# alehdaghi/vq-vae-2-pytorch

Measured on AMD Instinct MI355X. Metric: images/sec VQ-VAE-2 256px train step, higher is better.
Workload: dtype f32; 1 GPU; configs[1]: 256x256 FFHQ-shaped synthetic, default two-level VQ-VAE-2, batch 32/GPU; global_batch=32, image=256, n_embed=512, parallelism=dp1

## Files before the change

### vq-vae-2-pytorch_amd/csrc/vq2_resblock.hip

```cpp
#include "vq2_common.h"
#include "vq2_rbwino.h"

namespace vq2 {

typedef unsigned int u32x4 __attribute__((ext_vector_type(4)));

namespace rb {
constexpr unsigned RSRC_FLAGS = 0x00020000;
constexpr int OOB = 0x7F000000;
constexpr int TH = 8, TW = 16;
constexpr int PW = TW + 2, PH = TH + 2;
constexpr int NPATCH = PW * PH;
constexpr int CS = 16;
constexpr int LDK = CS + 4;
constexpr int CM = 32;
constexpr int CC = 128;
constexpr int A_F4 = NPATCH * CS / 4;
constexpr int B_F4 = 9 * CM * CS / 4;
constexpr int A_FLOATS = ((A_F4 + 255) / 256) * 64 * LDK;
constexpr int B_FLOATS = ((B_F4 + 255) / 256) * 64 * LDK;
constexpr int LDR = CM + 4;
constexpr size_t LDS_BYTES = (size_t)2 * (A_FLOATS + B_FLOATS) * sizeof(float);
static_assert(2 * LDS_BYTES <= 160 * 1024, "two workgroups per CU");
static_assert(128 * LDR <= 2 * (A_FLOATS + B_FLOATS), "stage-2 aliases fit in the stage-1 buffers");
}

struct ResFwdParams {
    const float *x;
    const float *w1;
    const float *b1;
    const float *w2;
    const float *b2;
    float *r;
    float *y;
    int N, H, W, ldx, ldr, ldy;
    int tiles_x, tiles_y;
    int relu_out;
};

__device__ __forceinline__ float4 u4_as_f4(u32x4 v) {
    return make_float4(__uint_as_float(v.x), __uint_as_float(v.y), __uint_as_float(v.z), __uint_as_float(v.w));
}

__global__ __launch_bounds__(256, 2) void resblock_fwd_kernel(const ResFwdParams P) {
    using namespace rb;
    constexpr int NT = 256;
    constexpr int A_LD = (A_F4 + NT - 1) / NT;
    constexpr int B_LD = (B_F4 + NT - 1) / NT;
    constexpr int NS = CC / CS;
    constexpr int NJ = CC / 32;
    extern __shared__ __attribute__((aligned(16))) float smem[];
    float *As = smem;
    float *Bs = smem + 2 * A_FLOATS;
    float *Rs = smem;

    const int tid = threadIdx.x, lane = tid & 63, wave = tid >> 6;
    const int wq = wave;
    const int l31 = lane & 31, fk = 4 * (lane >> 5);
    const int tiles = P.tiles_x * P.tiles_y;
    const int vid = xcd_remap(blockIdx.x, gridDim.x);
    const int n = vid / tiles;
    const int t = vid - n * tiles;
    const int tyi = t / P.tiles_x;
    const int y0 = tyi * TH, x0 = (t - tyi * P.tiles_x) * TW;

    const int npix = P.N * P.H * P.W;
    const __amdgpu_buffer_rsrc_t rx = __builtin_amdgcn_make_buffer_rsrc(const_cast<float *>(P.x), 0, npix * P.ldx * 4, RSRC_FLAGS);
    const __amdgpu_buffer_rsrc_t rw1 = __builtin_amdgcn_make_buffer_rsrc(const_cast<float *>(P.w1), 0, CM * 9 * CC * 4, RSRC_FLAGS);
    const __amdgpu_buffer_rsrc_t rw2 = __builtin_amdgcn_make_buffer_rsrc(const_cast<float *>(P.w2), 0, CC * CM * 4, RSRC_FLAGS);

    int a_off[A_LD], b_off[B_LD];
#pragma unroll
    for (int j = 0; j < A_LD; ++j) {
        const int f = tid + NT * j;
        a_off[j] = OOB;
        if (f < A_F4) {
            const int pp = f >> 2;
            const int pr = pp / PW, pc = pp - pr * PW;
            const int gy = y0 - 1 + pr, gx = x0 - 1 + pc;
            if ((unsigned)gy < (unsigned)P.H && (unsigned)gx < (unsigned)P.W)
                a_off[j] = ((n * P.H + gy) * P.W + gx) * P.ldx * 4 + (f & 3) * 16;
        }
    }
#pragma unroll
    for (int j = 0; j < B_LD; ++j) {
        const int f = tid + NT * j;
        b_off[j] = OOB;
        if (f < B_F4) {
            const int row = f >> 2;
            b_off[j] = ((row & 31) * 9 * CC + (row >> 5) * CC) * 4 + (f & 3) * 16;
        }
    }
    const int st_off = (tid >> 2) * LDK + (tid & 3) * 4;
    struct Slice { u32x4 a[A_LD], b[B_LD]; };
    auto issue_loads = [&](int s, Slice &r) {
        const int soff = s * CS * 4;
#pragma unroll
        for (int j = 0; j < A_LD; ++j) r.a[j] = __builtin_amdgcn_raw_buffer_load_b128(rx, a_off[j], soff, 0);
#pragma unroll
        for (int j = 0; j < B_LD; ++j) r.b[j] = __builtin_amdgcn_raw_buffer_load_b128(rw1, b_off[j], soff, 0);
    };
    auto store_slice = [&](int buf, const Slice &r) {
        float *a = As + buf * A_FLOATS + st_off;
        float *b = Bs + buf * B_FLOATS + st_off;
#pragma unroll
        for (int j = 0; j < A_LD; ++j)
            *reinterpret_cast<float4 *>(a + j * (NT / 4) * LDK) = relu4(u4_as_f4(r.a[j]));
#pragma unroll
        for (int j = 0; j < B_LD; ++j)
            *reinterpret_cast<float4 *>(b + j * (NT / 4) * LDK) = u4_as_f4(r.b[j]);
    };

    f32x16 acc1;
#pragma unroll
    for (int r = 0; r < 16; ++r) acc1[r] = 0.f;

    const int a_frag = ((2 * wq + (l31 >> 4)) * PW + (l31 < 16 ? l31 : ((l31 + 14) & 15))) * LDK + fk;
    const int b_frag = l31 * LDK + fk;
    auto stage_one_store = [&](int buf, const Slice &r, int j) {
        if (j < A_LD) *reinterpret_cast<float4 *>(As + buf * A_FLOATS + st_off + j * (NT / 4) * LDK) = relu4(u4_as_f4(r.a[j]));
        else *reinterpret_cast<float4 *>(Bs + buf * B_FLOATS + st_off + (j - A_LD) * (NT / 4) * LDK) = u4_as_f4(r.b[j - A_LD]);
    };
    auto stage_one_load = [&](int s, Slice &r, int j) {
        if (j < A_LD) r.a[j] = __builtin_amdgcn_raw_buffer_load_b128(rx, a_off[j], s * CS * 4, 0);
        else r.b[j - A_LD] = __builtin_amdgcn_raw_buffer_load_b128(rw1, b_off[j - A_LD], s * CS * 4, 0);
    };
    int pix_lane;
    {
        const int gy = y0 + 2 * wq + (l31 >> 4), gx = x0 + (l31 < 16 ? l31 : ((l31 + 14) & 15));
        pix_lane = (gy < P.H && gx < P.W) ? (n * P.H + gy) * P.W + gx : -1;
    }
    const int rowq = 4 * (lane >> 5);
    int xoff[16], yoff[16];
#pragma unroll
    for (int r = 0; r < 16; ++r) {
        const int pix = __shfl(pix_lane, rowq + (r & 3) + 8 * (r >> 2), 64);
        xoff[r] = pix >= 0 ? pix * (P.ldx * 4) + l31 * 4 : OOB;
        yoff[r] = pix >= 0 ? pix * (P.ldy * 4) + l31 * 4 : OOB;
    }
    f32x16 acc2[NJ];
    float4 w2f[NJ][CM / 8];
    float b1v = 0.f, b2v[NJ];
    const __amdgpu_buffer_rsrc_t rb1 = __builtin_amdgcn_make_buffer_rsrc(const_cast<float *>(P.b1), 0, CM * 4, RSRC_FLAGS);
    const __amdgpu_buffer_rsrc_t rb2 = __builtin_amdgcn_make_buffer_rsrc(const_cast<float *>(P.b2), 0, CC * 4, RSRC_FLAGS);

    auto stage2_load = [&](int i) {
        constexpr int NW2 = NJ * (CM / 8);
        if (i < NW2) {
            const int j = i / (CM / 8), k8 = i % (CM / 8);
            w2f[j][k8] = u4_as_f4(__builtin_amdgcn_raw_buffer_load_b128(rw2, ((j * 32 + l31) * CM + fk + 8 * k8) * 4, 0, 0));
        } else if (i < NW2 + NJ * 16) {
            const int j = (i - NW2) / 16, r = (i - NW2) % 16;
            acc2[j][r] = __uint_as_float(__builtin_amdgcn_raw_buffer_load_b32(rx, xoff[r] + j * 128, 0, 0));
        } else if (i == NW2 + NJ * 16) {
            b1v = __uint_as_float(__builtin_amdgcn_raw_buffer_load_b32(rb1, l31 * 4, 0, 0));
        } else if (i <= NW2 + NJ * 16 + NJ) {
            const int j = i - (NW2 + NJ * 16 + 1);
            b2v[j] = __uint_as_float(__builtin_amdgcn_raw_buffer_load_b32(rb2, (j * 32 + l31) * 4, 0, 0));
        }
    };
    auto compute_staged = [&](int buf, int s, Slice &r, bool do_store, bool do_load, bool do_stage2) {
        const float *a0 = As + buf * A_FLOATS + a_frag;
        const float *b0 = Bs + buf * B_FLOATS + b_frag;
        constexpr int NP = 9 * (CS / 8);
        constexpr int NST = A_LD + B_LD;
        static_assert(2 * NST <= NP, "stores then loads fit in the MFMA groups of one slice");
        float4 fa[2], fb[2];
        fa[0] = *reinterpret_cast<const float4 *>(a0);
        fb[0] = *reinterpret_cast<const float4 *>(b0);
#pragma unroll
        for (int p = 0; p < NP; ++p) {
            const int cur = p & 1, nxt = cur ^ 1;
            if (p + 1 < NP) {
                const int tap = (p + 1) / (CS / 8), k8 = (p + 1) % (CS / 8);
                fa[nxt] = *reinterpret_cast<const float4 *>(a0 + ((tap / 3) * PW + (tap % 3)) * LDK + 8 * k8);
                fb[nxt] = *reinterpret_cast<const float4 *>(b0 + tap * 32 * LDK + 8 * k8);
            }
            acc1 = __builtin_amdgcn_mfma_f32_32x32x2f32(fa[cur].x, fb[cur].x, acc1, 0, 0, 0);
            acc1 = __builtin_amdgcn_mfma_f32_32x32x2f32(fa[cur].y, fb[cur].y, acc1, 0, 0, 0);
            acc1 = __builtin_amdgcn_mfma_f32_32x32x2f32(fa[cur].z, fb[cur].z, acc1, 0, 0, 0);
            acc1 = __builtin_amdgcn_mfma_f32_32x32x2f32(fa[cur].w, fb[cur].w, acc1, 0, 0, 0);
            if (p < NST) { if (do_store) stage_one_store(buf ^ 1, r, p); }
            __builtin_amdgcn_sched_group_barrier(0x100, 2, 0);
            __builtin_amdgcn_sched_group_barrier(0x008, 4, 0);
            if (p < NST) __builtin_amdgcn_sched_group_barrier(0x200, 1, 0);
            if (p >= NST && p < 2 * NST && do_load) {
                __builtin_amdgcn_sched_barrier(0);
                stage_one_load(s + 2, r, p - NST);
                __builtin_amdgcn_sched_barrier(0);
            }
            if (do_stage2) {
                constexpr int PER = (NJ * (CM / 8) + NJ * 16 + 1 + NJ + NP - 1) / NP;
                __builtin_amdgcn_sched_barrier(0);
#pragma unroll
                for (int q = 0; q < PER; ++q) stage2_load(p * PER + q);
                __builtin_amdgcn_sched_barrier(0);
            }
        }
    };

    Slice R0, R1;
    issue_loads(0, R0);
    issue_loads(1, R1);
    store_slice(0, R0);
    __syncthreads();
    store_slice(1, R1);
    __builtin_amdgcn_sched_barrier(0);
    compute_staged(0, 0, R0, false, true, false);
    __builtin_amdgcn_sched_barrier(0);
    __syncthreads();
    for (int s = 1; s < NS; ++s) {
        const int buf = s & 1;
        __builtin_amdgcn_sched_barrier(0);
        compute_staged(buf, s, R0, s + 1 < NS, s + 2 < NS, s + 1 == NS);
        __builtin_amdgcn_sched_barrier(0);
        __syncthreads();
    }
    const __amdgpu_buffer_rsrc_t rr = __builtin_amdgcn_make_buffer_rsrc(P.r, 0, npix * P.ldr * 4, RSRC_FLAGS);
    const __amdgpu_buffer_rsrc_t ry = __builtin_amdgcn_make_buffer_rsrc(P.y, 0, npix * P.ldy * 4, RSRC_FLAGS);
    float rv[16];
    int roff[16];
    {
        const int ldr4 = P.ldr * 4;
#pragma unroll
        for (int r = 0; r < 16; ++r) {
            const int row = rowq + (r & 3) + 8 * (r >> 2);
            const int pix = __shfl(pix_lane, row, 64);
            rv[r] = relu1(acc1[r] + b1v);
            Rs[(32 * wq + row) * LDR + l31] = rv[r];
            roff[r] = pix >= 0 ? pix * ldr4 + l31 * 4 : OOB;
        }
    }
    const int relu_floor_bits = P.relu_out ? 0 : (int)0x80000000;
    {
        const float *a = Rs + (32 * wq + l31) * LDR + fk;
        float4 fa[CM / 8];
#pragma unroll
        for (int k8 = 0; k8 < CM / 8; ++k8) fa[k8] = *reinterpret_cast<const float4 *>(a + 8 * k8);
#pragma unroll
        for (int j = 0; j < NJ; ++j) {
#pragma unroll
            for (int r = 0; r < 16; ++r) acc2[j][r] += b2v[j];
#pragma unroll
            for (int k8 = 0; k8 < CM / 8; ++k8) {
                const float4 fb = w2f[j][k8];
                acc2[j] = __builtin_amdgcn_mfma_f32_32x32x2f32(fa[k8].x, fb.x, acc2[j], 0, 0, 0);
                acc2[j] = __builtin_amdgcn_mfma_f32_32x32x2f32(fa[k8].y, fb.y, acc2[j], 0, 0, 0);
                acc2[j] = __builtin_amdgcn_mfma_f32_32x32x2f32(fa[k8].z, fb.z, acc2[j], 0, 0, 0);
                acc2[j] = __builtin_amdgcn_mfma_f32_32x32x2f32(fa[k8].w, fb.w, acc2[j], 0, 0, 0);
                __builtin_amdgcn_sched_barrier(0);
#pragma unroll
                for (int q = 0; q < 4; ++q) {
                    const int r = 4 * k8 + q;
                    if (j == 0) {
                        __builtin_amdgcn_raw_buffer_store_b32(__float_as_uint(rv[r]), rr, roff[r], 0, 0);
                    } else {
                        const float v = relu_floor(acc2[j - 1][r], relu_floor_bits);
                        __builtin_amdgcn_raw_buffer_store_b32(__float_as_uint(v), ry, yoff[r] + (j - 1) * 128, 0, 0);
                    }
                }
                __builtin_amdgcn_sched_barrier(0);
            }
        }
    }
#pragma unroll
    for (int r = 0; r < 16; ++r) {
        const float v = relu_floor(acc2[NJ - 1][r], relu_floor_bits);
        __builtin_amdgcn_raw_buffer_store_b32(__float_as_uint(v), ry, yoff[r] + (NJ - 1) * 128, 0, 0);
    }
}


namespace rbb {
using namespace rb;
constexpr int SA = 32;
constexpr int LDA = SA + 4;
constexpr int PROWS = 192;
constexpr int GA_FLOATS = PROWS * LDA;
constexpr int WA_FLOATS = CM * LDA;
constexpr int WB_FLOATS = CC * LDA;
constexpr size_t LDS_BYTES = (size_t)(2 * GA_FLOATS + 2 * WA_FLOATS) * sizeof(float);
constexpr int WR_FLOATS = 16 * 64 + 32;
constexpr size_t LDS_BYTES_W2 = LDS_BYTES + (size_t)4 * WR_FLOATS * sizeof(float);
static_assert(GA_FLOATS + 2 * WB_FLOATS <= 2 * GA_FLOATS + 2 * WA_FLOATS, "phase-B buffers alias the phase-A ones");
}

struct ResBwdParams {
    const float *g;
    const float *r;
    const float *x;
    const float *w2d;
    const float *w1d;
    float *dh;
    float *dx;
    float *w2_slab;
    float *b2_slab;
    int N, H, W, ldg, ldr, ldx, lddh, lddx;
    int tiles_x, tiles_y;
};

template <bool SAME_LD>
__global__ __launch_bounds__(256, 2) void resblock_bwd_data_kernel(const ResBwdParams P) {
    using namespace rbb;
    extern __shared__ __attribute__((aligned(16))) float smem[];
    float *Ga = smem;
    float *Wa = smem + 2 * GA_FLOATS;
    float *Dh = smem;
    float *Wb = smem + GA_FLOATS;

    const int tid = threadIdx.x, lane = tid & 63, wq = tid >> 6;
    const int l31 = lane & 31, fk = 4 * (lane >> 5), rowq = 4 * (lane >> 5);
    const int tiles = P.tiles_x * P.tiles_y;
    const int vid = xcd_remap(blockIdx.x, gridDim.x);
    const int n = vid / tiles;
    const int t = vid - n * tiles;
    const int tyi = t / P.tiles_x;
    const int y0 = tyi * TH, x0 = (t - tyi * P.tiles_x) * TW;
    const int npix = P.N * P.H * P.W;
    const __amdgpu_buffer_rsrc_t rg = __builtin_amdgcn_make_buffer_rsrc(const_cast<float *>(P.g), 0, npix * P.ldg * 4, RSRC_FLAGS);
    const __amdgpu_buffer_rsrc_t rr = __builtin_amdgcn_make_buffer_rsrc(const_cast<float *>(P.r), 0, npix * P.ldr * 4, RSRC_FLAGS);
    const __amdgpu_buffer_rsrc_t rx = __builtin_amdgcn_make_buffer_rsrc(const_cast<float *>(P.x), 0, npix * P.ldx * 4, RSRC_FLAGS);
    const __amdgpu_buffer_rsrc_t rw2 = __builtin_amdgcn_make_buffer_rsrc(const_cast<float *>(P.w2d), 0, CM * CC * 4, RSRC_FLAGS);
    const __amdgpu_buffer_rsrc_t rw1 = __builtin_amdgcn_make_buffer_rsrc(const_cast<float *>(P.w1d), 0, CC * 9 * CM * 4, RSRC_FLAGS);

    auto patch_pix = [&](int pp) {
        const int pr = pp / PW, pc = pp - pr * PW;
        const int gy = y0 - 1 + pr, gx = x0 - 1 + pc;
        return (pp < NPATCH && (unsigned)gy < (unsigned)P.H && (unsigned)gx < (unsigned)P.W) ? (n * P.H + gy) * P.W + gx : -1;
    };

    constexpr int GA_LD = (NPATCH * (SA / 4) + 255) / 256;
    int ga_off[GA_LD];
#pragma unroll
    for (int j = 0; j < GA_LD; ++j) {
        const int f = tid + 256 * j;
        const int pix = patch_pix(f >> 3);
        ga_off[j] = pix >= 0 ? pix * P.ldg * 4 + (f & 7) * 16 : OOB;
    }
    const int wa_off = ((tid >> 3) * CC) * 4 + (tid & 7) * 16;
    const int st8 = (tid >> 3) * LDA + (tid & 7) * 4;
    constexpr int NSA = CC / SA;
    struct SliceA { u32x4 g[GA_LD], w; };
    auto issue_a = [&](int s, SliceA &r) {
        const int soff = s * SA * 4;
#pragma unroll
        for (int j = 0; j < GA_LD; ++j) r.g[j] = __builtin_amdgcn_raw_buffer_load_b128(rg, ga_off[j], soff, 0);
        r.w = __builtin_amdgcn_raw_buffer_load_b128(rw2, wa_off, soff, 0);
    };
    auto store_a = [&](int s, const SliceA &r) {
        const int buf = s & 1;
        float *a = Ga + buf * GA_FLOATS + st8;
#pragma unroll
        for (int j = 0; j < GA_LD; ++j) *reinterpret_cast<float4 *>(a + j * 32 * LDA) = u4_as_f4(r.g[j]);
        *reinterpret_cast<float4 *>(Wa + buf * WA_FLOATS + st8) = u4_as_f4(r.w);
    };
    static_assert(GA_LD * 256 == PROWS * (SA / 4), "the staging passes cover the padded patch exactly");
    const int nblk = wq < 2 ? 2 : 1;
    SliceA RA0, RA1;
    issue_a(0, RA0);
    issue_a(1, RA1);
    int pixA[2];
    float rmask[2][16];
#pragma unroll
    for (int bi = 0; bi < 2; ++bi) {
        pixA[bi] = patch_pix(32 * (wq + 4 * bi) + l31);
#pragma unroll
        for (int q = 0; q < 16; ++q) {
            const int pix = __shfl(pixA[bi], rowq + (q & 3) + 8 * (q >> 2), 64);
            rmask[bi][q] = __uint_as_float(__builtin_amdgcn_raw_buffer_load_b32(
                rr, (bi < nblk && pix >= 0) ? pix * P.ldr * 4 + l31 * 4 : OOB, 0, 0));
        }
    }
    f32x16 accA[2];
#pragma unroll
    for (int bi = 0; bi < 2; ++bi)
#pragma unroll
        for (int q = 0; q < 16; ++q) accA[bi][q] = 0.f;

    const bool fuse_w2 = P.w2_slab != nullptr;
    float *Wr = smem + 2 * GA_FLOATS + 2 * WA_FLOATS;
    float rB[16];
#pragma unroll
    for (int kk = 0; kk < 16; ++kk) {
        const int q = 2 * kk + (lane >> 5);
        const int gy = y0 + 2 * wq + (q >> 4), gx = x0 + (q & 15);
        const int pix = (gy < P.H && gx < P.W) ? (n * P.H + gy) * P.W + gx : -1;
        rB[kk] = __uint_as_float(__builtin_amdgcn_raw_buffer_load_b32(rr, (fuse_w2 && pix >= 0) ? pix * P.ldr * 4 + l31 * 4 : OOB, 0, 0));
    }
    const int wb_goff = ((tid >> 3) * 9 * CM) * 4 + (tid & 7) * 16;
    u32x4 rwb[4];
    auto issue_b = [&](int tap) {
#pragma unroll
        for (int j = 0; j < 4; ++j) rwb[j] = __builtin_amdgcn_raw_buffer_load_b128(rw1, wb_goff + j * 32 * 9 * CM * 4, tap * CM * 4, 0);
    };
    auto store_b = [&](int buf) {
#pragma unroll
        for (int j = 0; j < 4; ++j) *reinterpret_cast<float4 *>(Wb + buf * WB_FLOATS + st8 + j * 32 * LDA) = u4_as_f4(rwb[j]);
    };

    store_a(0, RA0);
    __syncthreads();
#pragma unroll
    for (int s = 0; s < NSA; ++s) {
        const int buf = s & 1;
        if (s + 1 < NSA) store_a(s + 1, s == 0 ? RA1 : RA0);
        if (s + 2 < NSA) issue_a(s + 2, RA0); else if (s + 2 == NSA) issue_b(0);
        __builtin_amdgcn_sched_barrier(0);
        {
            const float *b = Wa + buf * WA_FLOATS + l31 * LDA + fk;
#pragma unroll
            for (int bi = 0; bi < 2; ++bi) {
                if (bi < nblk) {
                    const float *a = Ga + buf * GA_FLOATS + (32 * (wq + 4 * bi) + l31) * LDA + fk;
#pragma unroll
                    for (int k8 = 0; k8 < SA / 8; ++k8) {
                        const float4 fa = *reinterpret_cast<const float4 *>(a + 8 * k8);
                        const float4 fb = *reinterpret_cast<const float4 *>(b + 8 * k8);
                        accA[bi] = __builtin_amdgcn_mfma_f32_32x32x2f32(fa.x, fb.x, accA[bi], 0, 0, 0);
                        accA[bi] = __builtin_amdgcn_mfma_f32_32x32x2f32(fa.y, fb.y, accA[bi], 0, 0, 0);
                        accA[bi] = __builtin_amdgcn_mfma_f32_32x32x2f32(fa.z, fb.z, accA[bi], 0, 0, 0);
                        accA[bi] = __builtin_amdgcn_mfma_f32_32x32x2f32(fa.w, fb.w, accA[bi], 0, 0, 0);
                    }
                }
            }
        }
        if (fuse_w2) {
            f32x16 aw;
#pragma unroll
            for (int r = 0; r < 16; ++r) aw[r] = 0.f;
            float bs = 0.f;
            const float *ga = Ga + buf * GA_FLOATS + l31;
#pragma unroll
            for (int kk = 0; kk < 16; ++kk) {
                const int q = 2 * kk + (lane >> 5);
                const float a = ga[((2 * wq + (q >> 4) + 1) * PW + (q & 15) + 1) * LDA];
                aw = __builtin_amdgcn_mfma_f32_32x32x2f32(a, rB[kk], aw, 0, 0, 0);
                bs += a;
            }
            float *wr = Wr + wq * WR_FLOATS;
#pragma unroll
            for (int r = 0; r < 16; ++r) wr[r * 64 + lane] = aw[r];
            bs += __shfl_xor(bs, 32, 64);
            if (lane < 32) wr[16 * 64 + lane] = bs;
        }
        __builtin_amdgcn_sched_barrier(0);
        __syncthreads();
        if (fuse_w2) {
            float *slab = P.w2_slab + ((size_t)blockIdx.x * CC + s * 32) * CM;
#pragma unroll
            for (int i = 0; i < 4; ++i) {
                const int r = 4 * wq + i;
                const float v = (Wr[r * 64 + lane] + Wr[WR_FLOATS + r * 64 + lane]) + (Wr[2 * WR_FLOATS + r * 64 + lane] + Wr[3 * WR_FLOATS + r * 64 + lane]);
                slab[(rowq + (r & 3) + 8 * (r >> 2)) * CM + l31] = v;
            }
            if (wq == 0 && lane < 32)
                P.b2_slab[(size_t)blockIdx.x * CC + s * 32 + lane] =
                    (Wr[16 * 64 + lane] + Wr[WR_FLOATS + 16 * 64 + lane]) + (Wr[2 * WR_FLOATS + 16 * 64 + lane] + Wr[3 * WR_FLOATS + 16 * 64 + lane]);
            __syncthreads();
        }
    }
    store_b(0);
    issue_b(1);
    {
        const __amdgpu_buffer_rsrc_t rdh = __builtin_amdgcn_make_buffer_rsrc(P.dh, 0, npix * P.lddh * 4, RSRC_FLAGS);
#pragma unroll
        for (int bi = 0; bi < 2; ++bi) {
            if (bi < nblk) {
                const int pp = 32 * (wq + 4 * bi) + l31;
                const int pr = pp / PW, pc = pp - pr * PW;
                const int own = (pr >= 1 && pr <= TH && pc >= 1 && pc <= TW) ? pixA[bi] : -1;
#pragma unroll
                for (int q = 0; q < 16; ++q) {
                    const int row = rowq + (q & 3) + 8 * (q >> 2);
                    const float v = rmask[bi][q] > 0.f ? accA[bi][q] : 0.f;
                    Dh[(32 * (wq + 4 * bi) + row) * LDA + l31] = v;
                    const int pix = __shfl(own, row, 64);
                    __builtin_amdgcn_raw_buffer_store_b32(__float_as_uint(v), rdh, pix >= 0 ? pix * P.lddh * 4 + l31 * 4 : OOB, 0, 0);
                }
            }
        }
    }
    __syncthreads();

    f32x16 acc[4];
#pragma unroll
    for (int j = 0; j < 4; ++j)
#pragma unroll
        for (int q = 0; q < 16; ++q) acc[j][q] = 0.f;
    const int txr = l31 < 16 ? l31 : ((l31 + 14) & 15);
    const int a_frag = ((2 * wq + (l31 >> 4)) * PW + txr) * LDA + fk;
    int poff[16];
    int pixr[SAME_LD ? 1 : 16];
    {
        const int gy = y0 + 2 * wq + (l31 >> 4), gx = x0 + txr;
        const int pix_lane = (gy < P.H && gx < P.W) ? (n * P.H + gy) * P.W + gx : -1;
#pragma unroll
        for (int q = 0; q < 16; ++q) {
            const int pix = __shfl(pix_lane, rowq + (q & 3) + 8 * (q >> 2), 64);
            poff[q] = pix >= 0 ? pix * (P.ldx * 4) + l31 * 4 : OOB;
            if (!SAME_LD) pixr[q] = pix;
        }
    }
    float mtmp[16], gres[4][16];
    unsigned mbits[2] = {0u, 0u};
    auto issue_b_one = [&](int tap, int j) {
        rwb[j] = __builtin_amdgcn_raw_buffer_load_b128(rw1, wb_goff + j * 32 * 9 * CM * 4, tap * CM * 4, 0);
    };
    auto store_b_one = [&](int buf, int j) {
        *reinterpret_cast<float4 *>(Wb + buf * WB_FLOATS + st8 + j * 32 * LDA) = u4_as_f4(rwb[j]);
    };
#pragma unroll
    for (int tap = 0; tap < 9; ++tap) {
        const int buf = tap & 1;
        __builtin_amdgcn_sched_barrier(0);
        {
            const float *a = Dh + a_frag + ((tap / 3) * PW + (tap % 3)) * LDA;
            const float *b = Wb + buf * WB_FLOATS + l31 * LDA + fk;
            float4 fa[2], fb[2];
            fa[0] = *reinterpret_cast<const float4 *>(a);
            fb[0] = *reinterpret_cast<const float4 *>(b);
#pragma unroll
            for (int g = 0; g < 16; ++g) {
                const int k8 = g >> 2, j = g & 3, cur = g & 1, nxt = cur ^ 1, ca = k8 & 1;
                if (g + 1 < 16) {
                    const int k8n = (g + 1) >> 2, jn = (g + 1) & 3;
                    fb[nxt] = *reinterpret_cast<const float4 *>(b + jn * 32 * LDA + 8 * k8n);
                    if (jn == 0) fa[k8n & 1] = *reinterpret_cast<const float4 *>(a + 8 * k8n);
                }
                acc[j] = __builtin_amdgcn_mfma_f32_32x32x2f32(fa[ca].x, fb[cur].x, acc[j], 0, 0, 0);
                acc[j] = __builtin_amdgcn_mfma_f32_32x32x2f32(fa[ca].y, fb[cur].y, acc[j], 0, 0, 0);
                acc[j] = __builtin_amdgcn_mfma_f32_32x32x2f32(fa[ca].z, fb[cur].z, acc[j], 0, 0, 0);
                acc[j] = __builtin_amdgcn_mfma_f32_32x32x2f32(fa[ca].w, fb[cur].w, acc[j], 0, 0, 0);
                if (g + 1 < 16) {
                    if (((g + 1) & 3) == 0) __builtin_amdgcn_sched_group_barrier(0x100, 2, 0);
                    else __builtin_amdgcn_sched_group_barrier(0x100, 1, 0);
                }
                __builtin_amdgcn_sched_group_barrier(0x008, 4, 0);
                __builtin_amdgcn_sched_barrier(0);
                if (g < 4 && tap + 1 < 9) store_b_one(buf ^ 1, g);
                if (g >= 4 && g < 8 && tap + 2 < 9) issue_b_one(tap + 2, g - 4);
                if (tap < 4 && g < 8) {
#pragma unroll
                    for (int q = 2 * g; q < 2 * g + 2; ++q)
                        mtmp[q] = __uint_as_float(__builtin_amdgcn_raw_buffer_load_b32(rx, poff[q], tap * 128, 0));
                }
                if (tap >= 5)
                    gres[tap - 5][g] = __uint_as_float(__builtin_amdgcn_raw_buffer_load_b32(
                        rg, SAME_LD ? poff[g] : (pixr[SAME_LD ? 0 : g] >= 0 ? pixr[SAME_LD ? 0 : g] * P.ldg * 4 + l31 * 4 : OOB),
                        (tap - 5) * 128, 0));
                __builtin_amdgcn_sched_barrier(0);
            }
        }
        __builtin_amdgcn_sched_barrier(0);
        if (tap < 4) {
#pragma unroll
            for (int q = 0; q < 16; ++q) mbits[tap >> 1] |= (mtmp[q] > 0.f ? 1u : 0u) << ((tap & 1) * 16 + q);
        }
        __syncthreads();
    }
    const __amdgpu_buffer_rsrc_t rdx = __builtin_amdgcn_make_buffer_rsrc(P.dx, 0, npix * P.lddx * 4, RSRC_FLAGS);
#pragma unroll
    for (int j = 0; j < 4; ++j)
#pragma unroll
        for (int q = 0; q < 16; ++q) {
            float v = ((mbits[j >> 1] >> ((j & 1) * 16 + q)) & 1u) ? acc[j][q] : 0.f;
            v += gres[j][q];
            __builtin_amdgcn_raw_buffer_store_b32(
                __float_as_uint(v), rdx,
                SAME_LD ? poff[q] : (pixr[SAME_LD ? 0 : q] >= 0 ? pixr[SAME_LD ? 0 : q] * P.lddx * 4 + l31 * 4 : OOB), j * 128, 0);
        }
}

}

extern "C" int vq2_resblock_supported(int32_t C, int32_t Cm) { return (C == vq2::rb::CC && Cm == vq2::rb::CM) ? 1 : 0; }

extern "C" int vq2_resblock_fwd(int32_t N, int32_t H, int32_t W, int32_t C, int32_t Cm, int flags, const float *x,
                                int32_t ldx, const float *w1p, const float *b1, const float *w2p, const float *b2,
                                float *r, int32_t ldr, float *y, int32_t ldy, vq2_stream_t stream) {
    using namespace vq2;
    VQ2_REQUIRE(N > 0 && H > 0 && W > 0, "resblock_fwd: empty tensor");
    if (int e = check_forms()) return e;
    if (!vq2_resblock_supported(C, Cm))
        return set_error(VQ2_ERR_UNSUPPORTED, "resblock_fwd: fused kernel is built for channel=%d, n_res_channel=%d (got %d, %d)",
                         rb::CC, rb::CM, C, Cm);
    VQ2_REQUIRE(x && w1p && b1 && w2p && b2 && r && y, "resblock_fwd: null pointer");
    VQ2_REQUIRE(aligned16(x) && aligned16(w1p) && aligned16(w2p) && aligned16(r) && aligned16(y),
                "resblock_fwd: pointers must be 16-byte aligned");
    VQ2_REQUIRE(ldx >= C && ldy >= C && ldr >= Cm && ldx % 4 == 0 && ldy % 4 == 0 && ldr % 4 == 0,
                "resblock_fwd: pixel strides must cover the channels and be multiples of 4");
    VQ2_REQUIRE((flags & ~VQ2_RELU_OUT) == 0, "resblock_fwd: only VQ2_RELU_OUT is a valid flag");
    const double npix = (double)N * H * W;
    const int ldmax = ldx > ldy ? ldx : ldy;
    VQ2_REQUIRE(npix * ldmax * 4.0 < (double)rb::OOB, "resblock_fwd: tensors must be smaller than %d bytes", rb::OOB);
    {
        RbwFwdParams Q{};
        Q.x = x; Q.w1 = w1p; Q.b1 = b1; Q.w2 = w2p; Q.b2 = b2; Q.r = r; Q.y = y;
        Q.N = N; Q.H = H; Q.W = W; Q.ldx = ldx; Q.ldr = ldr; Q.ldy = ldy; Q.relu_out = (flags & VQ2_RELU_OUT) != 0;
        if (ldr >= Cm && rbw_fwd_ok(Q)) {
            hipStream_t s = to_stream(stream);
            const char *name = "resblock_fwd_wino";
            if (prof_enabled()) name = prof_label("resblock_fwd_wino|M=%d,C=%d,Cm=%d", N * H * W, C, Cm);
            ProfScope prof(name, 2.0 * npix * (9.0 * C * Cm + (double)Cm * C), 4.0 * npix * (2.0 * C + Cm), s);
            return launch_rbw_fwd(Q, s);
        }
    }
    ResFwdParams P{};
    P.x = x; P.w1 = w1p; P.b1 = b1; P.w2 = w2p; P.b2 = b2; P.r = r; P.y = y;
    P.N = N; P.H = H; P.W = W; P.ldx = ldx; P.ldr = ldr; P.ldy = ldy;
    P.tiles_x = (W + rb::TW - 1) / rb::TW; P.tiles_y = (H + rb::TH - 1) / rb::TH;
    P.relu_out = (flags & VQ2_RELU_OUT) != 0;
    const int grid = N * P.tiles_x * P.tiles_y;
    hipStream_t s = to_stream(stream);
    const char *name = "resblock_fwd";
    if (prof_enabled()) name = prof_label("resblock_fwd|M=%d,C=%d,Cm=%d", N * H * W, C, Cm);
    ProfScope prof(name, 2.0 * npix * (9.0 * C * Cm + (double)Cm * C), 4.0 * npix * (2.0 * C + Cm), s);
    allow_big_lds(resblock_fwd_kernel, rb::LDS_BYTES);
    hipLaunchKernelGGL(resblock_fwd_kernel, dim3(grid), dim3(256), rb::LDS_BYTES, s, P);
    return check_launch("resblock_fwd_kernel");
}

static int rb_grid(int N, int H, int W) { return N * ((W + vq2::rb::TW - 1) / vq2::rb::TW) * ((H + vq2::rb::TH - 1) / vq2::rb::TH); }

extern "C" size_t vq2_resblock_w2_workspace_bytes(int32_t N, int32_t H, int32_t W, int32_t C, int32_t Cm) {
    if (N <= 0 || H <= 0 || W <= 0 || !vq2_resblock_supported(C, Cm)) return 0;
    return (size_t)rb_grid(N, H, W) * ((size_t)C * Cm + C) * sizeof(float);
}

extern "C" int vq2_resblock_w2_job_init(int32_t N, int32_t H, int32_t W, int32_t C, int32_t Cm, const void *ws, float *dw,
                                        float *db, vq2_wgrad_job *job) {
    VQ2_REQUIRE(ws && dw && job && vq2_resblock_supported(C, Cm) && N > 0 && H > 0 && W > 0, "resblock_w2_job_init: bad arguments");
    const int S = rb_grid(N, H, W);
    const float *w = static_cast<const float *>(ws);
    job->ws = w; job->dw = dw; job->bias_ws = db ? w + (size_t)S * C * Cm : nullptr; job->db = db;
    job->unit_offset = 0;
    job->O = C; job->I = Cm; job->Or = C; job->Ir = Cm; job->taps = 1; job->S = S;
    job->n_units_w = (C * Cm + 31) / 32; job->n_units_b = db ? (C + 31) / 32 : 0;
    job->swapped = 0; job->bias_splits = 0;
    return VQ2_OK;
}

extern "C" int vq2_resblock_bwd_data(int32_t N, int32_t H, int32_t W, int32_t C, int32_t Cm, const float *g, int32_t ldg,
                                     const float *r, int32_t ldr, const float *x, int32_t ldx, const float *w2d,
                                     const float *w1d, float *dh, int32_t lddh, float *dx, int32_t lddx, void *w2_ws,
                                     vq2_stream_t stream) {
    using namespace vq2;
    VQ2_REQUIRE(N > 0 && H > 0 && W > 0, "resblock_bwd_data: empty tensor");
    if (!vq2_resblock_supported(C, Cm))
        return set_error(VQ2_ERR_UNSUPPORTED, "resblock_bwd_data: fused kernel is built for channel=%d, n_res_channel=%d (got %d, %d)",
                         rb::CC, rb::CM, C, Cm);
    VQ2_REQUIRE(g && r && x && w2d && w1d && dh && dx, "resblock_bwd_data: null pointer");
    VQ2_REQUIRE(aligned16(g) && aligned16(r) && aligned16(x) && aligned16(w2d) && aligned16(w1d) && aligned16(dh) && aligned16(dx),
                "resblock_bwd_data: pointers must be 16-byte aligned");
    VQ2_REQUIRE(ldg >= C && ldx >= C && lddx >= C && ldr >= Cm && lddh >= Cm && ldg % 4 == 0 && ldx % 4 == 0 &&
                    lddx % 4 == 0 && ldr % 4 == 0 && lddh % 4 == 0,
                "resblock_bwd_data: pixel strides must cover the channels and be multiples of 4");
    const double npix = (double)N * H * W;
    int ldmax = ldg > ldx ? ldg : ldx;
    if (lddx > ldmax) ldmax = lddx;
    VQ2_REQUIRE(npix * ldmax * 4.0 < (double)rb::OOB, "resblock_bwd_data: tensors must be smaller than %d bytes", rb::OOB);
    ResBwdParams P{};
    P.g = g; P.r = r; P.x = x; P.w2d = w2d; P.w1d = w1d; P.dh = dh; P.dx = dx;
    VQ2_REQUIRE(!w2_ws || aligned16(w2_ws), "resblock_bwd_data: workspace must be 16-byte aligned");
    P.N = N; P.H = H; P.W = W; P.ldg = ldg; P.ldr = ldr; P.ldx = ldx; P.lddh = lddh; P.lddx = lddx;
    P.tiles_x = (W + rb::TW - 1) / rb::TW; P.tiles_y = (H + rb::TH - 1) / rb::TH;
    const int grid = N * P.tiles_x * P.tiles_y;
    hipStream_t s = to_stream(stream);
    const char *name = "resblock_bwd_data";
    if (prof_enabled()) name = prof_label("resblock_bwd_data|M=%d,C=%d,Cm=%d", N * H * W, C, Cm);
    ProfScope prof(name, 2.0 * npix * (9.0 * C * Cm + (double)Cm * C), 4.0 * npix * (4.0 * C + 2.0 * Cm), s);
    P.w2_slab = static_cast<float *>(w2_ws);
    P.b2_slab = w2_ws ? P.w2_slab + (size_t)grid * C * Cm : nullptr;
    const size_t lds = w2_ws ? rbb::LDS_BYTES_W2 : rbb::LDS_BYTES;
    if (ldg == ldx && lddx == ldx) {
        allow_big_lds(resblock_bwd_data_kernel<true>, lds);
        hipLaunchKernelGGL(resblock_bwd_data_kernel<true>, dim3(grid), dim3(256), lds, s, P);
    } else {
        allow_big_lds(resblock_bwd_data_kernel<false>, lds);
        hipLaunchKernelGGL(resblock_bwd_data_kernel<false>, dim3(grid), dim3(256), lds, s, P);
    }
    return check_launch("resblock_bwd_data_kernel");
}
```

Measured before the change: 5481 images/s.

## Add Winograd F(2,3) path for resblock backward-data 3x3 convolution

Adds a resblock backward-data kernel that computes the transposed 3x3 convolution with Winograd F(2,3) along the width axis. Weight-side transforms (g0, g0+g1+g2, g0-g1+g2, g2) are built while staging into LDS, and the input-side transform runs in registers before the MFMAs, which cuts the multiply count for the 3x3 taps. The shared phase A (1x1 gradient and w2 slab) is factored into a helper templated on the phase-B prefetch hooks, so both kernels reuse it. The new path is taken only when FORMS_ALL is set and H and W are multiples of the tile size. It adds extra adds and some rounding differences, plus a different LDS layout and register pressure.

```diff
diff --git a/vq-vae-2-pytorch_amd/csrc/vq2_resblock.hip b/vq-vae-2-pytorch_amd/csrc/vq2_resblock.hip
--- a/vq-vae-2-pytorch_amd/csrc/vq2_resblock.hip
+++ b/vq-vae-2-pytorch_amd/csrc/vq2_resblock.hip
@@ -299,14 +299,12 @@
     int tiles_x, tiles_y;
 };
 
-template <bool SAME_LD>
-__global__ __launch_bounds__(256, 2) void resblock_bwd_data_kernel(const ResBwdParams P) {
+template <class PrefetchB, class HandoverB>
+__device__ __forceinline__ void rbb_phase_a(const ResBwdParams &P, float *smem, PrefetchB &&prefetch_b, HandoverB &&handover_b) {
     using namespace rbb;
-    extern __shared__ __attribute__((aligned(16))) float smem[];
     float *Ga = smem;
     float *Wa = smem + 2 * GA_FLOATS;
     float *Dh = smem;
-    float *Wb = smem + GA_FLOATS;
 
     const int tid = threadIdx.x, lane = tid & 63, wq = tid >> 6;
     const int l31 = lane & 31, fk = 4 * (lane >> 5), rowq = 4 * (lane >> 5);
@@ -319,9 +317,7 @@
     const int npix = P.N * P.H * P.W;
     const __amdgpu_buffer_rsrc_t rg = __builtin_amdgcn_make_buffer_rsrc(const_cast<float *>(P.g), 0, npix * P.ldg * 4, RSRC_FLAGS);
     const __amdgpu_buffer_rsrc_t rr = __builtin_amdgcn_make_buffer_rsrc(const_cast<float *>(P.r), 0, npix * P.ldr * 4, RSRC_FLAGS);
-    const __amdgpu_buffer_rsrc_t rx = __builtin_amdgcn_make_buffer_rsrc(const_cast<float *>(P.x), 0, npix * P.ldx * 4, RSRC_FLAGS);
     const __amdgpu_buffer_rsrc_t rw2 = __builtin_amdgcn_make_buffer_rsrc(const_cast<float *>(P.w2d), 0, CM * CC * 4, RSRC_FLAGS);
-    const __amdgpu_buffer_rsrc_t rw1 = __builtin_amdgcn_make_buffer_rsrc(const_cast<float *>(P.w1d), 0, CC * 9 * CM * 4, RSRC_FLAGS);
 
     auto patch_pix = [&](int pp) {
         const int pr = pp / PW, pc = pp - pr * PW;
@@ -387,24 +383,13 @@
         const int pix = (gy < P.H && gx < P.W) ? (n * P.H + gy) * P.W + gx : -1;
         rB[kk] = __uint_as_float(__builtin_amdgcn_raw_buffer_load_b32(rr, (fuse_w2 && pix >= 0) ? pix * P.ldr * 4 + l31 * 4 : OOB, 0, 0));
     }
-    const int wb_goff = ((tid >> 3) * 9 * CM) * 4 + (tid & 7) * 16;
-    u32x4 rwb[4];
-    auto issue_b = [&](int tap) {
-#pragma unroll
-        for (int j = 0; j < 4; ++j) rwb[j] = __builtin_amdgcn_raw_buffer_load_b128(rw1, wb_goff + j * 32 * 9 * CM * 4, tap * CM * 4, 0);
-    };
-    auto store_b = [&](int buf) {
-#pragma unroll
-        for (int j = 0; j < 4; ++j) *reinterpret_cast<float4 *>(Wb + buf * WB_FLOATS + st8 + j * 32 * LDA) = u4_as_f4(rwb[j]);
-    };
-
     store_a(0, RA0);
     __syncthreads();
 #pragma unroll
     for (int s = 0; s < NSA; ++s) {
         const int buf = s & 1;
         if (s + 1 < NSA) store_a(s + 1, s == 0 ? RA1 : RA0);
-        if (s + 2 < NSA) issue_a(s + 2, RA0); else if (s + 2 == NSA) issue_b(0);
+        if (s + 2 < NSA) issue_a(s + 2, RA0); else if (s + 2 == NSA) prefetch_b();
         __builtin_amdgcn_sched_barrier(0);
         {
             const float *b = Wa + buf * WA_FLOATS + l31 * LDA + fk;
@@ -459,8 +444,7 @@
             __syncthreads();
         }
     }
-    store_b(0);
-    issue_b(1);
+    handover_b();
     {
         const __amdgpu_buffer_rsrc_t rdh = __builtin_amdgcn_make_buffer_rsrc(P.dh, 0, npix * P.lddh * 4, RSRC_FLAGS);
 #pragma unroll
@@ -481,6 +465,40 @@
         }
     }
     __syncthreads();
+}
+
+template <bool SAME_LD>
+__global__ __launch_bounds__(256, 2) void resblock_bwd_data_kernel(const ResBwdParams P) {
+    using namespace rbb;
+    extern __shared__ __attribute__((aligned(16))) float smem[];
+    float *Dh = smem;
+    float *Wb = smem + GA_FLOATS;
+
+    const int tid = threadIdx.x, lane = tid & 63, wq = tid >> 6;
+    const int l31 = lane & 31, fk = 4 * (lane >> 5), rowq = 4 * (lane >> 5);
+    const int tiles = P.tiles_x * P.tiles_y;
+    const int vid = xcd_remap(blockIdx.x, gridDim.x);
+    const int n = vid / tiles;
+    const int t = vid - n * tiles;
+    const int tyi = t / P.tiles_x;
+    const int y0 = tyi * TH, x0 = (t - tyi * P.tiles_x) * TW;
+    const int npix = P.N * P.H * P.W;
+    const __amdgpu_buffer_rsrc_t rg = __builtin_amdgcn_make_buffer_rsrc(const_cast<float *>(P.g), 0, npix * P.ldg * 4, RSRC_FLAGS);
+    const __amdgpu_buffer_rsrc_t rx = __builtin_amdgcn_make_buffer_rsrc(const_cast<float *>(P.x), 0, npix * P.ldx * 4, RSRC_FLAGS);
+    const __amdgpu_buffer_rsrc_t rw1 = __builtin_amdgcn_make_buffer_rsrc(const_cast<float *>(P.w1d), 0, CC * 9 * CM * 4, RSRC_FLAGS);
+    const int st8 = (tid >> 3) * LDA + (tid & 7) * 4;
+    const int wb_goff = ((tid >> 3) * 9 * CM) * 4 + (tid & 7) * 16;
+    u32x4 rwb[4];
+    auto issue_b = [&](int tap) {
+#pragma unroll
+        for (int j = 0; j < 4; ++j) rwb[j] = __builtin_amdgcn_raw_buffer_load_b128(rw1, wb_goff + j * 32 * 9 * CM * 4, tap * CM * 4, 0);
+    };
+    auto store_b = [&](int buf) {
+#pragma unroll
+        for (int j = 0; j < 4; ++j) *reinterpret_cast<float4 *>(Wb + buf * WB_FLOATS + st8 + j * 32 * LDA) = u4_as_f4(rwb[j]);
+    };
+
+    rbb_phase_a(P, smem, [&] { issue_b(0); }, [&] { store_b(0); issue_b(1); });
 
     f32x16 acc[4];
 #pragma unroll
@@ -569,6 +587,153 @@
                 __float_as_uint(v), rdx,
                 SAME_LD ? poff[q] : (pixr[SAME_LD ? 0 : q] >= 0 ? pixr[SAME_LD ? 0 : q] * P.lddx * 4 + l31 * 4 : OOB), j * 128, 0);
         }
+}
+
+namespace rbbw {
+using namespace rbb;
+constexpr int KS = 16;
+constexpr int LDU = KS + 4;
+constexpr int CH = 64;
+constexpr int NPASS = CC / CH;
+constexpr int NBLK = 3 * (CM / KS);
+constexpr int U_FLOATS = 4 * CH * LDU;
+constexpr size_t LDS_B = (size_t)(GA_FLOATS + 2 * U_FLOATS) * sizeof(float);
+constexpr size_t LDS_BYTES = LDS_B > rbb::LDS_BYTES ? LDS_B : rbb::LDS_BYTES;
+constexpr size_t LDS_BYTES_W2 = rbb::LDS_BYTES_W2;
+static_assert(LDS_B <= rbb::LDS_BYTES_W2, "phase B fits in what phase A with the 1x1 weight gradient allocates");
+static_assert(CH * (KS / 4) == 256, "one (ci, quad) item of a panel block per thread");
+}
+
+__global__ __launch_bounds__(256, 2) void resblock_bwd_wino_kernel(const ResBwdParams P) {
+    using namespace rbbw;
+    extern __shared__ __attribute__((aligned(16))) float smem[];
+    float *Dh = smem;
+    float *Us = smem + GA_FLOATS;
+
+    const int tid = threadIdx.x, lane = tid & 63, wq = tid >> 6;
+    const int l31 = lane & 31, fk = 4 * (lane >> 5), rowq = 4 * (lane >> 5);
+    const int tiles = P.tiles_x * P.tiles_y;
+    const int vid = xcd_remap(blockIdx.x, gridDim.x);
+    const int n = vid / tiles;
+    const int t = vid - n * tiles;
+    const int tyi = t / P.tiles_x;
+    const int y0 = tyi * TH, x0 = (t - tyi * P.tiles_x) * TW;
+    const int npix = P.N * P.H * P.W;
+    const __amdgpu_buffer_rsrc_t rg = __builtin_amdgcn_make_buffer_rsrc(const_cast<float *>(P.g), 0, npix * P.ldg * 4, RSRC_FLAGS);
+    const __amdgpu_buffer_rsrc_t rx = __builtin_amdgcn_make_buffer_rsrc(const_cast<float *>(P.x), 0, npix * P.ldx * 4, RSRC_FLAGS);
+    const __amdgpu_buffer_rsrc_t rw1 = __builtin_amdgcn_make_buffer_rsrc(const_cast<float *>(P.w1d), 0, CC * 9 * CM * 4, RSRC_FLAGS);
+
+    const int u_goff = ((tid >> 2) * 9 * CM) * 4 + (tid & 3) * 16;
+    const int u_dst = (tid >> 2) * LDU + (tid & 3) * 4;
+    u32x4 ru[3];
+    auto load_u = [&](int b) {
+        const int pass = b / NBLK, kh = (b % NBLK) >> 1, half = b & 1;
+        const int soff = ((pass * CH * 9 + kh * 3) * CM + half * KS) * 4;
+#pragma unroll
+        for (int kw = 0; kw < 3; ++kw) ru[kw] = __builtin_amdgcn_raw_buffer_load_b128(rw1, u_goff, soff + kw * CM * 4, 0);
+    };
+    auto store_u = [&](int buf) {
+        float *u = Us + buf * U_FLOATS + u_dst;
+        const float4 g0 = u4_as_f4(ru[0]), g1 = u4_as_f4(ru[1]), g2 = u4_as_f4(ru[2]);
+        const float4 s = make_float4(g0.x + g2.x, g0.y + g2.y, g0.z + g2.z, g0.w + g2.w);
+        *reinterpret_cast<float4 *>(u + 0 * CH * LDU) = g0;
+        *reinterpret_cast<float4 *>(u + 1 * CH * LDU) = make_float4(s.x + g1.x, s.y + g1.y, s.z + g1.z, s.w + g1.w);
+        *reinterpret_cast<float4 *>(u + 2 * CH * LDU) = make_float4(s.x - g1.x, s.y - g1.y, s.z - g1.z, s.w - g1.w);
+        *reinterpret_cast<float4 *>(u + 3 * CH * LDU) = g2;
+    };
+    rbb_phase_a(P, smem, [&] { load_u(0); }, [&] { store_u(0); load_u(1); });
+
+    const int wr = wq & 1, wc = wq >> 1;
+    const int a_frag = ((4 * wr + (l31 >> 3)) * PW + 2 * (l31 & 7)) * LDA + fk;
+    const int b_frag = (32 * wc + l31) * LDU + fk;
+    const int pix_lane = (n * P.H + y0 + 4 * wr) * P.W + x0 + 2 * rowq;
+    const int ch_lane = (32 * wc + l31) * 4;
+    const int xbase = pix_lane * (P.ldx * 4) + ch_lane, gbase = pix_lane * (P.ldg * 4) + ch_lane, dxbase = pix_lane * (P.lddx * 4) + ch_lane;
+    auto pix_of = [&](int q, int px) { return (q >> 2) * P.W + 2 * (q & 3) + px; };
+    const __amdgpu_buffer_rsrc_t rdx = __builtin_amdgcn_make_buffer_rsrc(P.dx, 0, npix * P.lddx * 4, RSRC_FLAGS);
+
+    float4 d[2][4], fb[2][4];
+    auto read_step = [&](const float *a, const float *b, int set) {
+#pragma unroll
+        for (int c = 0; c < 4; ++c) d[set][c] = *reinterpret_cast<const float4 *>(a + c * LDA);
+#pragma unroll
+        for (int v = 0; v < 4; ++v) fb[set][v] = *reinterpret_cast<const float4 *>(b + v * CH * LDU);
+    };
+    auto sub4 = [](float4 a, float4 b) { return make_float4(a.x - b.x, a.y - b.y, a.z - b.z, a.w - b.w); };
+    auto add4 = [](float4 a, float4 b) { return make_float4(a.x + b.x, a.y + b.y, a.z + b.z, a.w + b.w); };
+
+#pragma unroll
+    for (int pass = 0; pass < NPASS; ++pass) {
+        f32x16 acc[4];
+#pragma unroll
+        for (int v = 0; v < 4; ++v)
+#pragma unroll
+            for (int q = 0; q < 16; ++q) acc[v][q] = 0.f;
+        float mtmp[16], gres[2][16];
+        unsigned mbits = 0u;
+#pragma unroll
+        for (int s = 0; s < NBLK; ++s) {
+            const int b = pass * NBLK + s, buf = b & 1;
+            const int kh = s >> 1, half = s & 1;
+            if (b >= 1 && b + 1 < NPASS * NBLK) load_u(b + 1);
+            __builtin_amdgcn_sched_barrier(0);
+            const float *a = Dh + a_frag + kh * PW * LDA + half * KS;
+            const float *bp = Us + buf * U_FLOATS + b_frag;
+            read_step(a, bp, 0);
+            __builtin_amdgcn_sched_group_barrier(0x100, 8, 0);
+#pragma unroll
+            for (int k8 = 0; k8 < KS / 8; ++k8) {
+                const int cur = k8 & 1;
+                if (k8 + 1 < KS / 8) read_step(a + 8 * (k8 + 1), bp + 8 * (k8 + 1), cur ^ 1);
+                float4 fv[4];
+                fv[0] = sub4(d[cur][0], d[cur][2]);
+                fv[1] = add4(d[cur][1], d[cur][2]);
+                fv[2] = sub4(d[cur][2], d[cur][1]);
+                fv[3] = sub4(d[cur][1], d[cur][3]);
+#define VQ2_RBBW_STEP(C) \
+    _Pragma("unroll") for (int v = 0; v < 4; ++v) acc[v] = __builtin_amdgcn_mfma_f32_32x32x2f32(fv[v].C, fb[cur][v].C, acc[v], 0, 0, 0);
+                VQ2_RBBW_STEP(x) VQ2_RBBW_STEP(y) VQ2_RBBW_STEP(z) VQ2_RBBW_STEP(w)
+#undef VQ2_RBBW_STEP
+                if (k8 + 1 < KS / 8) __builtin_amdgcn_sched_group_barrier(0x100, 8, 0);
+                __builtin_amdgcn_sched_group_barrier(0x002, 16, 0);
+                __builtin_amdgcn_sched_group_barrier(0x008, 16, 0);
+                __builtin_amdgcn_sched_barrier(0);
+                const int slot = 2 * s + k8;
+                if (slot < 2 || (slot >= 4 && slot < 6)) {
+                    const int px = slot >> 2;
+#pragma unroll
+                    for (int q = 8 * (slot & 1); q < 8 * (slot & 1) + 8; ++q)
+                        mtmp[q] = __uint_as_float(__builtin_amdgcn_raw_buffer_load_b32(rx, xbase, pix_of(q, px) * (P.ldx * 4) + pass * CH * 4, 0));
+                }
+                if (slot >= 6 && slot < 10) {
+                    const int px = (slot - 6) >> 1;
+#pragma unroll
+                    for (int q = 8 * (slot & 1); q < 8 * (slot & 1) + 8; ++q)
+                        gres[px][q] = __uint_as_float(__builtin_amdgcn_raw_buffer_load_b32(rg, gbase, pix_of(q, px) * (P.ldg * 4) + pass * CH * 4, 0));
+                }
+                __builtin_amdgcn_sched_barrier(0);
+            }
+            if (s == 1 || s == 3) {
+                const int px = s >> 1;
+#pragma unroll
+                for (int q = 0; q < 16; ++q) mbits |= (mtmp[q] > 0.f ? 1u : 0u) << (16 * px + q);
+            }
+            if (b + 1 < NPASS * NBLK) store_u(buf ^ 1);
+            __syncthreads();
+        }
+#pragma unroll
+        for (int q = 0; q < 16; ++q) {
+            const float m0 = acc[0][q], m1 = acc[1][q], m2 = acc[2][q], m3 = acc[3][q];
+            float v0 = m0 + 0.5f * (m1 + m2);
+            float v1 = 0.5f * (m1 - m2) - m3;
+            v0 = ((mbits >> q) & 1u) ? v0 : 0.f;
+            v1 = ((mbits >> (16 + q)) & 1u) ? v1 : 0.f;
+            v0 += gres[0][q];
+            v1 += gres[1][q];
+            __builtin_amdgcn_raw_buffer_store_b32(__float_as_uint(v0), rdx, dxbase, pix_of(q, 0) * (P.lddx * 4) + pass * CH * 4, 0);
+            __builtin_amdgcn_raw_buffer_store_b32(__float_as_uint(v1), rdx, dxbase, pix_of(q, 1) * (P.lddx * 4) + pass * CH * 4, 0);
+        }
+    }
 }
 
 }
@@ -666,11 +831,19 @@
     P.tiles_x = (W + rb::TW - 1) / rb::TW; P.tiles_y = (H + rb::TH - 1) / rb::TH;
     const int grid = N * P.tiles_x * P.tiles_y;
     hipStream_t s = to_stream(stream);
+    P.w2_slab = static_cast<float *>(w2_ws);
+    P.b2_slab = w2_ws ? P.w2_slab + (size_t)grid * C * Cm : nullptr;
     const char *name = "resblock_bwd_data";
+    if (forms() == FORMS_ALL && W % rb::TW == 0 && H % rb::TH == 0) {
+        if (prof_enabled()) name = prof_label("resblock_bwd_data<wino>|M=%d,C=%d,Cm=%d", N * H * W, C, Cm);
+        ProfScope prof(name, 2.0 * npix * (9.0 * C * Cm + (double)Cm * C), 4.0 * npix * (4.0 * C + 2.0 * Cm), s);
+        const size_t lds = w2_ws ? rbbw::LDS_BYTES_W2 : rbbw::LDS_BYTES;
+        allow_big_lds(resblock_bwd_wino_kernel, lds);
+        hipLaunchKernelGGL(resblock_bwd_wino_kernel, dim3(grid), dim3(256), lds, s, P);
+        return check_launch("resblock_bwd_wino_kernel");
+    }
     if (prof_enabled()) name = prof_label("resblock_bwd_data|M=%d,C=%d,Cm=%d", N * H * W, C, Cm);
     ProfScope prof(name, 2.0 * npix * (9.0 * C * Cm + (double)Cm * C), 4.0 * npix * (4.0 * C + 2.0 * Cm), s);
-    P.w2_slab = static_cast<float *>(w2_ws);
-    P.b2_slab = w2_ws ? P.w2_slab + (size_t)grid * C * Cm : nullptr;
     const size_t lds = w2_ws ? rbb::LDS_BYTES_W2 : rbb::LDS_BYTES;
     if (ldg == ldx && lddx == ldx) {
         allow_big_lds(resblock_bwd_data_kernel<true>, lds);
```

Result: slower. 4960 images/s (-9.5%).
